# Cognoscan/entropy_coders

Hardware: AMD Instinct MI355X
Metric: FSE encode+decode GiB/s on 1 GiB synthetic bytes; bit-exact round-trip (higher is better)
Workload: dtype u8

## Files before the change

entropy_coders_amd/csrc/fse_decode.hip:

```cpp
#include <type_traits>
#include <utility>

#include "fse_device.hpp"
#include "fse_kernels.h"


namespace fsehip {

__device__ uint32_t g_rank_fb_dec;
hipError_t rank_fallbacks_dec(uint32_t* out, bool reset) {
    hipError_t e = hipMemcpyFromSymbol(out, HIP_SYMBOL(g_rank_fb_dec), 4, 0, hipMemcpyDeviceToHost);
    if (e == hipSuccess && reset) {
        const uint32_t z = 0;
        e = hipMemcpyToSymbol(HIP_SYMBOL(g_rank_fb_dec), &z, 4, 0, hipMemcpyHostToDevice);
    }
    return e;
}

constexpr int STAGE_AUX = 2;

template <int LMAX>
struct Dte {
    static constexpr uint32_t SH = LMAX > 14 ? 17u : 18u;
    __device__ static __forceinline__ uint32_t make(uint32_t nb, uint32_t sym, uint32_t ns) {
        return nb | (sym << 8) | (ns << SH);
    }
    __device__ static __forceinline__ uint32_t ns(uint32_t e) { return e >> SH; }
};
__device__ __forceinline__ uint32_t dte_nb(uint32_t e) { return e & 0xFFu; }
__device__ __forceinline__ uint32_t dte_sym(uint32_t e) { return (e >> 8) & 0xFFu; }

constexpr uint32_t DEC_GROUP = 32;

struct WindowReader {
    const uint32_t* w;
    uint64_t buf;
    int32_t base;
    int32_t pos;
    __device__ __forceinline__ void init(const uint32_t* words, int32_t p) {
        w = words;
        pos = p;
        base = ((p + 31) & ~31) - 64;
        if (base < 0) base = 0;
        buf = (uint64_t)w[base >> 5] | ((uint64_t)w[(base >> 5) + 1] << 32);
    }
    __device__ __forceinline__ uint32_t pop(uint32_t nb) {
        pos -= (int32_t)nb;
        return (uint32_t)(buf >> (uint32_t)(pos - base)) & ((1u << nb) - 1u);
    }
    __device__ __forceinline__ void refill() {
        if (pos - base < 32 && base > 0) {
            base -= 32;
            buf = (buf << 32) | (uint64_t)w[base >> 5];
        }
    }
};

__device__ __forceinline__ bool ckpt_match(uint64_t e, int32_t hdr_bits, uint32_t smask, int32_t pos, uint32_t a0,
                                           uint32_t a1) {
    return (int32_t)(uint32_t)e + hdr_bits == pos && ((((uint32_t)(e >> 32) & smask) << 2) == a0) &&
           ((((uint32_t)(e >> 48) & smask) << 2) == a1);
}

template <int LMAX, class Ent, class Pop>
__device__ __forceinline__ int32_t finish2(uint32_t o, uint32_t n, uint32_t& s0, uint32_t& s1, int32_t& pos,
                                           int32_t hdr_bits, uint8_t* __restrict__ out, Ent ent, Pop pop) {
    for (;;) {
        if (o + 2u == n) {
            out[o++] = (uint8_t)dte_sym(ent(s0));
            out[o++] = (uint8_t)dte_sym(ent(s1));
            break;
        }
        if (o + 1u == n) {
            out[o++] = (uint8_t)dte_sym(ent(s0));
            break;
        }
        const uint32_t e0 = ent(s0);
        uint32_t nb = dte_nb(e0);
        if (pos - (int32_t)nb < hdr_bits) {
            out[o++] = (uint8_t)dte_sym(e0);
            if (o < n) out[o++] = (uint8_t)dte_sym(ent(s1));
            break;
        }
        s0 = Dte<LMAX>::ns(e0) + pop(nb);
        out[o++] = (uint8_t)dte_sym(e0);
        const uint32_t e1 = ent(s1);
        nb = dte_nb(e1);
        if (pos - (int32_t)nb < hdr_bits) {
            out[o++] = (uint8_t)dte_sym(e1);
            if (o < n) out[o++] = (uint8_t)dte_sym(ent(s0));
            break;
        }
        s1 = Dte<LMAX>::ns(e1) + pop(nb);
        out[o++] = (uint8_t)dte_sym(e1);
    }
    return o != n ? FSE_ERR_LENGTH_MISMATCH : pos == hdr_bits ? FSE_OK : FSE_ERR_BAD_SIDECAR;
}

template <int LMAX>
__device__ __forceinline__ int32_t decode_segment(WindowReader& br, uint32_t& s0, uint32_t& s1, uint32_t p0,
                                                  uint32_t p1, bool last, uint32_t n, uint32_t Pm,
                                                  uint8_t* __restrict__ out, const uint32_t* dt, int32_t hdr_bits) {
    uint32_t p = p0;
    for (; p + 8u <= p1; p += 8u) {
        uint32_t w[4];
#pragma unroll
        for (int j = 0; j < 8; ++j) {
            const uint32_t e0 = dt[s0], e1 = dt[s1];
            const uint32_t v0 = br.pop(dte_nb(e0));
            const uint32_t v1 = br.pop(dte_nb(e1));
            s0 = Dte<LMAX>::ns(e0) + v0;
            s1 = Dte<LMAX>::ns(e1) + v1;
            const uint32_t pr = __builtin_amdgcn_perm(e1, e0, 0x0c0c0501u);
            if (j & 1) w[j >> 1] |= pr << 16; else w[j >> 1] = pr;
            br.refill();
        }
        *reinterpret_cast<uint4*>(out + 2u * p) = make_uint4(w[0], w[1], w[2], w[3]);
    }
    for (; p < p1; ++p) {
        const uint32_t e0 = dt[s0], e1 = dt[s1];
        const uint32_t v0 = br.pop(dte_nb(e0));
        const uint32_t v1 = br.pop(dte_nb(e1));
        s0 = Dte<LMAX>::ns(e0) + v0;
        s1 = Dte<LMAX>::ns(e1) + v1;
        out[2u * p] = (uint8_t)dte_sym(e0);
        out[2u * p + 1u] = (uint8_t)dte_sym(e1);
        br.refill();
    }
    if (!last) return FSE_OK;
    return finish2<LMAX>(2u * Pm, n, s0, s1, br.pos, hdr_bits, out, [&](uint32_t s) { return dt[s]; },
                         [&](uint32_t nb) {
                             const uint32_t v = br.pop(nb);
                             br.refill();
                             return v;
                         });
}

template <int LMAX>
__device__ __forceinline__ int32_t decode_segment1(WindowReader& br, uint32_t& s, uint32_t p, uint32_t p1, bool last,
                                                   uint32_t n, uint8_t* __restrict__ out, const uint32_t* dt,
                                                   int32_t hdr_bits) {
    for (; p < p1; ++p) {
        const uint32_t e = dt[s];
        s = Dte<LMAX>::ns(e) + br.pop(dte_nb(e));
        br.refill();
        out[p] = (uint8_t)dte_sym(e);
    }
    if (!last) return FSE_OK;
    out[n - 1u] = (uint8_t)dte_sym(dt[s]);
    return br.pos == hdr_bits ? FSE_OK : FSE_ERR_BAD_SIDECAR;
}

constexpr int32_t PAIR_MAX_BITS = 28;
struct LdsChain {
    int32_t pos, B;
    uint32_t whi, wlo, a0, a1;
    __device__ __forceinline__ void init(const uint32_t* pay, int32_t p, uint32_t s0, uint32_t s1) {
        pos = p;
        a0 = s0 << 2;
        a1 = s1 << 2;
        B = (p - PAIR_MAX_BITS) & ~31;
        wlo = 0;
        whi = *reinterpret_cast<const uint32_t*>(reinterpret_cast<const uint8_t*>(pay) + (B >> 3) + 4);
    }
    __device__ __forceinline__ uint32_t pair(const uint32_t* pay, const uint8_t* dtb) {
        const int32_t lo = (pos - PAIR_MAX_BITS) & ~31;
        const uint32_t w0 = *reinterpret_cast<const uint32_t*>(reinterpret_cast<const uint8_t*>(pay) + (lo >> 3));
        const uint32_t e0 = *reinterpret_cast<const uint32_t*>(dtb + a0);
        const uint32_t e1 = *reinterpret_cast<const uint32_t*>(dtb + a1);
        const uint32_t w1 = lo == B ? whi : wlo;
        pos -= (int32_t)((e0 + e1) & 0xFFu);
        const uint32_t x = (uint32_t)((((uint64_t)w1 << 32) | w0) >> (uint32_t)(pos - lo));
        B = lo;
        whi = w1;
        wlo = w0;
        const uint32_t v1 = __builtin_amdgcn_ubfe(x, 0u, e1);
        const uint32_t v0 = __builtin_amdgcn_ubfe(x, e1, e0);
        a0 = (e0 >> 16) + (v0 << 2);
        a1 = (e1 >> 16) + (v1 << 2);
        return __builtin_amdgcn_perm(e1, e0, 0x0c0c0501u);
    }
    __device__ __forceinline__ uint32_t s0() const { return a0 >> 2; }
    __device__ __forceinline__ uint32_t s1() const { return a1 >> 2; }
    __device__ static __forceinline__ uint32_t entry(const uint8_t* dtb, uint32_t s) {
        return *reinterpret_cast<const uint32_t*>(dtb + 4u * s);
    }
};
template <class Chain, class Tab>
__device__ __forceinline__ uint32_t two_pairs(Chain& c, const uint32_t* pay, const Tab& dtb) {
    const uint32_t lo = c.pair(pay, dtb);
    const uint32_t hi = c.pair(pay, dtb);
    return __builtin_amdgcn_perm(hi, lo, 0x05040100u);
}
__device__ __forceinline__ uint32_t lds_bits32(const uint32_t* pay, int32_t pos) {
    const uint32_t* wp = pay + ((uint32_t)pos >> 5);
    return __builtin_amdgcn_alignbit(wp[1], wp[0], (uint32_t)pos);
}

__device__ __forceinline__ void store_group(uint8_t* __restrict__ dst, const uint32_t* w) {
    uint4* o4 = reinterpret_cast<uint4*>(dst);
#pragma unroll
    for (uint32_t q = 0; q < DEC_GROUP / 8u; ++q) o4[q] = make_uint4(w[4 * q], w[4 * q + 1], w[4 * q + 2], w[4 * q + 3]);
}

__device__ __forceinline__ void rows_transpose(uint32_t* w) {
#pragma unroll
    for (int c = 0; c < 2; ++c)
#pragma unroll
        for (int d = 0; d < 4; ++d) {
            const auto r = __builtin_amdgcn_permlane32_swap(w[4 * c + d], w[4 * (c + 2) + d], false, false);
            w[4 * c + d] = r[0];
            w[4 * (c + 2) + d] = r[1];
        }
#pragma unroll
    for (int c = 0; c < 4; c += 2)
#pragma unroll
        for (int d = 0; d < 4; ++d) {
            const auto r = __builtin_amdgcn_permlane16_swap(w[4 * c + d], w[4 * (c + 1) + d], false, false);
            w[4 * c + d] = r[0];
            w[4 * (c + 1) + d] = r[1];
        }
}

template <class Chain, class Tab>
__device__ __forceinline__ void run_groups_tx(Chain& c, uint32_t my_ng, uint32_t ng_max, const uint32_t* pay,
                                              const Tab& dtb, uint8_t* const* obase, const uint32_t* ong,
                                              uint32_t row) {
    for (uint32_t g = 0; g < ng_max; ++g) {
        uint32_t w[DEC_GROUP / 2u];
        if (g < my_ng) {
#pragma unroll
            for (uint32_t j = 0; j < DEC_GROUP; j += 2u) w[j >> 1] = two_pairs(c, pay, dtb);
        } else {
#pragma unroll
            for (uint32_t j = 0; j < DEC_GROUP / 2u; ++j) w[j] = 0;
        }
        rows_transpose(w);
#pragma unroll
        for (int k = 0; k < 4; ++k)
            if (g < ong[k])
                __builtin_nontemporal_store(u32x4{w[4 * k], w[4 * k + 1], w[4 * k + 2], w[4 * k + 3]},
                                            reinterpret_cast<u32x4*>(obase[k] + g * 2u * DEC_GROUP + 16u * row));
    }
}

template <class Chain, class Tab>
__device__ __forceinline__ void run_chains2(Chain& a, Chain& b, const uint32_t* pay, const Tab& dtb, uint32_t pa,
                                            uint32_t pb, uint32_t ng, uint8_t* __restrict__ out) {
    for (uint32_t g = 0; g < ng; ++g) {
        uint32_t wa[DEC_GROUP / 2u], wb[DEC_GROUP / 2u];
#pragma unroll
        for (uint32_t j = 0; j < DEC_GROUP; j += 2u) {
            const uint32_t la = a.pair(pay, dtb);
            const uint32_t lb = b.pair(pay, dtb);
            const uint32_t ha = a.pair(pay, dtb);
            const uint32_t hb = b.pair(pay, dtb);
            wa[j >> 1] = __builtin_amdgcn_perm(ha, la, 0x05040100u);
            wb[j >> 1] = __builtin_amdgcn_perm(hb, lb, 0x05040100u);
        }
        store_group(out + 2u * (pa + g * DEC_GROUP), wa);
        store_group(out + 2u * (pb + g * DEC_GROUP), wb);
    }
}

template <class Chain, class Tab>
__device__ __forceinline__ int32_t run_chain(Chain& c, const uint32_t* pay, const Tab& dtb, uint32_t p, uint32_t p1,
                                             bool last, uint32_t n, uint32_t Pm, uint8_t* __restrict__ out,
                                             int32_t hdr_bits) {
    for (; p + DEC_GROUP <= p1; p += DEC_GROUP) {
        uint32_t w[DEC_GROUP / 2u];
#pragma unroll
        for (uint32_t j = 0; j < DEC_GROUP; j += 2u) w[j >> 1] = two_pairs(c, pay, dtb);
        store_group(out + 2u * p, w);
    }
    for (; p < p1; ++p) {
        const uint32_t pr = c.pair(pay, dtb);
        out[2u * p] = (uint8_t)pr;
        out[2u * p + 1u] = (uint8_t)(pr >> 8);
    }
    if (!last) return FSE_OK;
    uint32_t s0 = c.s0(), s1 = c.s1();
    return finish2<11>(2u * Pm, n, s0, s1, c.pos, hdr_bits, out, [&](uint32_t s) { return Chain::entry(dtb, s); },
                       [&](uint32_t nb) {
                           c.pos -= (int32_t)nb;
                           return __builtin_amdgcn_ubfe(lds_bits32(pay, c.pos), 0u, nb);
                       });
}

struct LdsChain1 {
    int32_t pos;
    uint32_t Q, whi, wlo, a;
    __device__ __forceinline__ void init(const uint32_t* pay, int32_t p, uint32_t s) {
        pos = p;
        a = s << 2;
        Q = ((uint32_t)p >> 3) & ~3u;
        wlo = 0;
        whi = *reinterpret_cast<const uint32_t*>(reinterpret_cast<const uint8_t*>(pay) + Q);
    }
    __device__ __forceinline__ uint32_t window(const uint32_t* pay) {
        const uint32_t q = ((uint32_t)pos >> 3) & ~3u;
        const uint32_t wq = *reinterpret_cast<const uint32_t*>(reinterpret_cast<const uint8_t*>(pay) + q - 4u);
        const uint32_t hi = q == Q ? whi : wlo;
        Q = q;
        whi = hi;
        wlo = wq;
        return __builtin_amdgcn_alignbit(hi, wq, (uint32_t)pos);
    }
    __device__ __forceinline__ uint32_t step(const uint32_t* pay, const uint8_t* dtb) {
        const uint32_t e = *reinterpret_cast<const uint32_t*>(dtb + a);
        const uint32_t x = window(pay);
        pos -= (int32_t)(e & 0xFFu);
        a = (e >> 16) + (__builtin_amdgcn_ubfe(x, 0u - e, e) << 2);
        return e;
    }
    __device__ __forceinline__ uint32_t pair(const uint32_t* pay, const uint8_t* dtb) {
        const uint32_t e0 = *reinterpret_cast<const uint32_t*>(dtb + a);
        const uint32_t x = window(pay);
        const uint32_t o0 = 0u - e0;
        const uint32_t a1 = (e0 >> 16) + (__builtin_amdgcn_ubfe(x, o0, e0) << 2);
        const uint32_t e1 = *reinterpret_cast<const uint32_t*>(dtb + a1);
        a = (e1 >> 16) + (__builtin_amdgcn_ubfe(x, o0 - e1, e1) << 2);
        pos -= (int32_t)((e0 + e1) & 0xFFu);
        return __builtin_amdgcn_perm(e1, e0, 0x0c0c0501u);
    }
};
struct Chain1x2 {
    LdsChain1 c;
    __device__ __forceinline__ uint32_t pair(const uint32_t* pay, const uint8_t* dtb) { return c.pair(pay, dtb); }
};

__device__ __forceinline__ int32_t run_chain1(LdsChain1& c, const uint32_t* pay, const uint8_t* dtb, uint32_t p,
                                              uint32_t p1, bool last, uint32_t n, uint8_t* __restrict__ out,
                                              int32_t hdr_bits) {
    constexpr uint32_t G = 2u * DEC_GROUP;
    for (; p + G <= p1; p += G) {
        uint32_t w[G / 4u];
#pragma unroll
        for (uint32_t j = 0; j < G; j += 4u) {
            const uint32_t lo = c.pair(pay, dtb), hi = c.pair(pay, dtb);
            w[j >> 2] = __builtin_amdgcn_perm(hi, lo, 0x05040100u);
        }
        uint4* o4 = reinterpret_cast<uint4*>(out + p);
#pragma unroll
        for (uint32_t q = 0; q < G / 16u; ++q) o4[q] = make_uint4(w[4 * q], w[4 * q + 1], w[4 * q + 2], w[4 * q + 3]);
    }
    for (; p < p1; ++p) out[p] = (uint8_t)dte_sym(c.step(pay, dtb));
    if (!last) return FSE_OK;
    out[n - 1u] = (uint8_t)dte_sym(*reinterpret_cast<const uint32_t*>(dtb + c.a));
    return c.pos == hdr_bits ? FSE_OK : FSE_ERR_BAD_SIDECAR;
}

template <uint32_t NT = 256u>
__device__ __forceinline__ uint32_t seg_of(uint32_t tid) {
    return (tid * 33u) & (NT - 1u);
}

template <int LMAX, uint32_t PMAX, uint32_t NW = 4u>
struct PreSmem {
    uint32_t pad[4];
    uint32_t pay[PMAX / 4];
    uint32_t dt[1u << LMAX];
    int err[NW];
};

template <int LMAX, uint32_t PMAX, int NS, uint32_t NT, class Smem>
__device__ __forceinline__ void decode_pre_block(const DecParams& P, Smem& sm, const uint64_t gb) {
    constexpr bool BIG = LMAX > 14;
    constexpr uint32_t NW = NT / 64u;
    const uint32_t tid = threadIdx.x, lane = tid & 63u, wv = tid >> 6;
    if (gb >= P.n_blocks) return;
    const uint8_t* in = P.in + gb * P.slot_bytes;
    const uint32_t clen = P.comp_len[gb];
    const uint64_t ooff = gb * (uint64_t)P.block_size;
    const uint32_t n = (uint32_t)min((uint64_t)P.block_size, P.n_total - ooff);
    uint8_t* out = P.out + ooff;
    const int32_t info = P.dtinfo[gb];
    const bool in_lds = !BIG && clen <= PMAX;
    if (P.pass >= 2 && P.status[gb] != FSE_DEFERRED) return;
    FSE_STAMP(P, 0);
    if (info < 0 || n < (NS == 2 ? 2u : 1u)) {
        if (tid == 0) P.status[gb] = info < 0 ? info : FSE_ERR_LENGTH_MISMATCH;
        return;
    }
    if ((P.pass == 1 || P.pass == 3) && !in_lds) {
        if (tid == 0) P.status[gb] = FSE_DEFERRED;
        return;
    }
    const int32_t hdr_bits = (info & 0xFFFF) * 8;
    const uint32_t L = (uint32_t)info >> 16;
    {
        if (in_lds) {
            const uint32_t nvec = (clen + 15u) >> 4;
            const uint4* src4 = reinterpret_cast<const uint4*>(in);
            uint4* dst4 = reinterpret_cast<uint4*>(sm.pay);
            for (uint32_t i = wv * 64u; i < nvec; i += NT)
                if (i + lane < nvec) __builtin_amdgcn_global_load_lds(src4 + i + lane, dst4 + i, 16, 0, STAGE_AUX);
        }
        {
            const uint32_t dvec = 1u << L >> 2;
            const uint4* t4 = reinterpret_cast<const uint4*>(P.dt + gb * (uint64_t)(1u << LMAX));
            uint4* d4 = reinterpret_cast<uint4*>(sm.dt);
            for (uint32_t i = wv * 64u; i < dvec; i += NT)
                if (i + lane < dvec) __builtin_amdgcn_global_load_lds(t4 + i + lane, d4 + i, 16, 0, STAGE_AUX);
        }
        asm volatile("s_waitcnt vmcnt(0)" ::: "memory");
        __syncthreads();
    }
    FSE_STAMP(P, 3);
    const uint32_t smask = (1u << L) - 1u;
    const uint32_t Pm = NS == 2 ? ((n & 1u) ? (n - 3u) / 2u : n / 2u - 1u) : n - 1u;
    const uint32_t I = P.ckpt_interval;
    const uint32_t nseg = Pm / I + 1u;
    const uint64_t* sc = P.sidecar + gb * P.ckpt_per_block;
    const uint32_t maxbp = clen * 8u - (uint32_t)hdr_bits;
    using Chain = LdsChain;
    const uint8_t* dtb = reinterpret_cast<const uint8_t*>(sm.dt);
    const uint32_t* gw = reinterpret_cast<const uint32_t*>(in);
    int32_t err = FSE_OK;
    uint32_t base0 = 0;
    if (NS == 2 && !BIG && in_lds && NT <= 256u) {
        for (; base0 + NT < nseg; base0 += 2u * NT) {
            const uint32_t sa = base0 + seg_of<NT>(tid), sb = sa + NT;
            bool act[2] = {sa < nseg, sb < nseg};
            const uint32_t sg[2] = {sa, sb};
            Chain c[2];
            uint32_t pp[2], pe[2];
            uint64_t en[2];
            int32_t r[2] = {FSE_OK, FSE_OK};
#pragma unroll
            for (int k = 0; k < 2; ++k) {
                pp[k] = sg[k] * I;
                pe[k] = min(pp[k] + I, Pm);
                en[k] = 0;
                if (!act[k]) continue;
                const uint64_t e = sc[sg[k]];
                en[k] = sg[k] == nseg - 1u ? 0ull : sc[sg[k] + 1u];
                if ((uint32_t)e > maxbp) {
                    r[k] = FSE_ERR_BAD_SIDECAR;
                    act[k] = false;
                    continue;
                }
                c[k].init(sm.pay, hdr_bits + (int32_t)(uint32_t)e, (uint32_t)(e >> 32) & smask,
                          (uint32_t)(e >> 48) & smask);
            }
            const uint32_t ng = (act[0] && act[1]) ? min(pe[0] - pp[0], pe[1] - pp[1]) / DEC_GROUP : 0u;
            run_chains2(c[0], c[1], sm.pay, dtb, pp[0], pp[1], ng, out);
#pragma unroll
            for (int k = 0; k < 2; ++k) {
                if (!act[k]) continue;
                const bool last = sg[k] == nseg - 1u;
                r[k] = run_chain(c[k], sm.pay, dtb, pp[k] + ng * DEC_GROUP, pe[k], last, n, Pm, out, hdr_bits);
                if (r[k] == FSE_OK && !last &&
                    !ckpt_match(en[k], hdr_bits, smask, c[k].pos, c[k].s0() << 2, c[k].s1() << 2))
                    r[k] = FSE_ERR_BAD_SIDECAR;
            }
            if (r[0] != FSE_OK) err = r[0];
            if (r[1] != FSE_OK) err = r[1];
        }
    }
    if (NS == 2 && !BIG && in_lds) {
        for (; base0 < nseg; base0 += NT) {
            const uint32_t seg = base0 + seg_of<NT>(tid);
            bool act = seg < nseg;
            const uint32_t p0 = seg * I, p1 = act ? min(p0 + I, Pm) : p0;
            const bool lastseg = seg == nseg - 1u;
            int32_t r = FSE_OK;
            Chain c;
            uint64_t en = 0;
            if (act) {
                const uint64_t e = sc[seg];
                en = lastseg ? 0ull : sc[seg + 1u];
                if ((uint32_t)e > maxbp) {
                    r = FSE_ERR_BAD_SIDECAR;
                    act = false;
                } else {
                    c.init(sm.pay, hdr_bits + (int32_t)(uint32_t)e, (uint32_t)(e >> 32) & smask,
                           (uint32_t)(e >> 48) & smask);
                }
            }
            const uint32_t my_ng = act ? (p1 - p0) / DEC_GROUP : 0u;
            const uint32_t ng_max = wave_max(my_ng);
            if (ng_max) {
                uint8_t* obase[4];
                uint32_t ong[4];
#pragma unroll
                for (uint32_t k = 0; k < 4; ++k) {
                    const uint32_t os = base0 + seg_of<NT>((tid & ~63u) + 16u * k + (tid & 15u));
                    const uint32_t oq = os * I;
                    ong[k] = os < nseg ? (min(oq + I, Pm) - oq) / DEC_GROUP : 0u;
                    obase[k] = out + 2u * oq;
                }
                run_groups_tx(c, my_ng, ng_max, sm.pay, dtb, obase, ong, (tid >> 4) & 3u);
            }
            if (act) {
                r = run_chain(c, sm.pay, dtb, p0 + my_ng * DEC_GROUP, p1, lastseg, n, Pm, out, hdr_bits);
                if (r == FSE_OK && !lastseg && !ckpt_match(en, hdr_bits, smask, c.pos, c.s0() << 2, c.s1() << 2))
                    r = FSE_ERR_BAD_SIDECAR;
            }
            if (r != FSE_OK) err = r;
        }
    }
    if (NS == 1 && !BIG && in_lds) {
        constexpr uint32_t G1 = 2u * DEC_GROUP;
        for (; base0 < nseg; base0 += NT) {
            const uint32_t seg = base0 + seg_of<NT>(tid);
            bool act = seg < nseg;
            const uint32_t p0 = seg * I, p1 = act ? min(p0 + I, Pm) : p0;
            const bool lastseg = seg == nseg - 1u;
            int32_t r = FSE_OK;
            Chain1x2 c;
            uint64_t en = 0;
            if (act) {
                const uint64_t e = sc[seg];
                en = lastseg ? 0ull : sc[seg + 1u];
                if ((uint32_t)e > maxbp) {
                    r = FSE_ERR_BAD_SIDECAR;
                    act = false;
                } else {
                    c.c.init(sm.pay, hdr_bits + (int32_t)(uint32_t)e, (uint32_t)(e >> 32) & smask);
                }
            }
            const uint32_t my_ng = act ? (p1 - p0) / G1 : 0u;
            const uint32_t ng_max = wave_max(my_ng);
            if (ng_max) {
                uint8_t* obase[4];
                uint32_t ong[4];
#pragma unroll
                for (uint32_t k = 0; k < 4; ++k) {
                    const uint32_t os = base0 + seg_of<NT>((tid & ~63u) + 16u * k + (tid & 15u));
                    const uint32_t oq = os * I;
                    ong[k] = os < nseg ? (min(oq + I, Pm) - oq) / G1 : 0u;
                    obase[k] = out + oq;
                }
                run_groups_tx(c, my_ng, ng_max, sm.pay, dtb, obase, ong, (tid >> 4) & 3u);
            }
            if (act) {
                r = run_chain1(c.c, sm.pay, dtb, p0 + my_ng * G1, p1, lastseg, n, out, hdr_bits);
                if (r == FSE_OK && !lastseg && !ckpt_match(en, hdr_bits, smask, c.c.pos, c.c.a, 0u))
                    r = FSE_ERR_BAD_SIDECAR;
            }
            if (r != FSE_OK) err = r;
        }
    }
    for (uint32_t base = base0; base < nseg; base += NT) {
        const uint32_t seg = base + (NS == 2 ? seg_of<NT>(tid) : tid);
        if (seg >= nseg) continue;
        const uint64_t e = sc[seg];
        const uint32_t p0 = seg * I, p1 = min(p0 + I, Pm);
        const uint32_t bp = (uint32_t)e;
        uint32_t s0 = (uint32_t)(e >> 32) & smask, s1 = NS == 2 ? (uint32_t)(e >> 48) & smask : 0u;
        const bool lastseg = seg == nseg - 1u;
        const uint64_t en = lastseg ? 0ull : sc[seg + 1u];
        int32_t r;
        if (bp > maxbp) {
            r = FSE_ERR_BAD_SIDECAR;
        } else if (NS == 1) {
            if (!BIG && in_lds) {
                LdsChain1 c;
                c.init(sm.pay, hdr_bits + (int32_t)bp, s0);
                r = run_chain1(c, sm.pay, dtb, p0, p1, lastseg, n, out, hdr_bits);
                if (r == FSE_OK && !lastseg && !ckpt_match(en, hdr_bits, smask, c.pos, c.a, 0u)) r = FSE_ERR_BAD_SIDECAR;
            } else {
                WindowReader br;
                br.init(gw, hdr_bits + (int32_t)bp);
                r = decode_segment1<LMAX>(br, s0, p0, p1, lastseg, n, out, sm.dt, hdr_bits);
                if (r == FSE_OK && !lastseg && !ckpt_match(en, hdr_bits, smask, br.pos, s0 << 2, 0u))
                    r = FSE_ERR_BAD_SIDECAR;
            }
        } else if (!BIG && in_lds) {
            Chain c;
            c.init(sm.pay, hdr_bits + (int32_t)bp, s0, s1);
            r = run_chain(c, sm.pay, dtb, p0, p1, lastseg, n, Pm, out, hdr_bits);
            if (r == FSE_OK && !lastseg && !ckpt_match(en, hdr_bits, smask, c.pos, c.a0, c.a1)) r = FSE_ERR_BAD_SIDECAR;
        } else {
            WindowReader br;
            br.init(gw, hdr_bits + (int32_t)bp);
            r = decode_segment<LMAX>(br, s0, s1, p0, p1, lastseg, n, Pm, out, sm.dt, hdr_bits);
            if (r == FSE_OK && !lastseg && !ckpt_match(en, hdr_bits, smask, br.pos, s0 << 2, s1 << 2))
                r = FSE_ERR_BAD_SIDECAR;
        }
        if (r != FSE_OK) err = r;
    }
    err = -(int32_t)wave_max((uint32_t)(-err));
    if (lane == 0) sm.err[wv] = err;
    __syncthreads();
    FSE_STAMP(P, 4);
    if (tid == 0) {
        int32_t e2 = FSE_OK;
        for (uint32_t w = 0; w < NW; ++w)
            if (sm.err[w] != FSE_OK) e2 = sm.err[w];
        P.status[gb] = e2;
        if (P.out_len) P.out_len[gb] = e2 ? 0u : n;
    }
}

template <int LMAX, uint32_t PMAX, int NS, int PASS, uint32_t NT = 256u>
__global__ __launch_bounds__(NT) void decode_pre_kernel(DecParams P) {
    constexpr bool BIG = LMAX > 14;
    constexpr uint32_t NW = NT / 64u;
    __shared__ PreSmem<LMAX, BIG ? 16u : PMAX, NW> sm;
    if constexpr (PASS <= 1) {
        decode_pre_block<LMAX, PMAX, NS, NT>(P, sm, blockIdx.x);
    } else {
        __shared__ uint64_t dmask[NW];
        const uint32_t tid = threadIdx.x, lane = tid & 63u, wv = tid >> 6;
        const uint64_t G = gridDim.x;
        for (uint64_t r0 = blockIdx.x; r0 < P.n_blocks; r0 += G * NT) {
            const uint64_t gb = r0 + G * tid;
            const bool d = gb < P.n_blocks && P.status[gb] == FSE_DEFERRED;
            const uint64_t m = __ballot(d);
            if (lane == 0) dmask[wv] = m;
            __syncthreads();
            for (uint32_t w = 0; w < NW; ++w) {
                for (uint64_t mw = dmask[w]; mw; mw &= mw - 1u)
                    decode_pre_block<LMAX, PMAX, NS, NT>(P, sm, r0 + G * (64u * w + (uint32_t)__builtin_ctzll(mw)));
            }
            __syncthreads();
        }
    }
}

constexpr uint32_t HP_BLOCKS = 16;
template <int LMAX>
__global__ __launch_bounds__(64) void hdr_parse_kernel(DtParams P) {
    static_assert(LMAX <= 12, "headers of L <= 12 fit the 512 staged bytes");
    constexpr uint32_t NB = HP_BLOCKS;
    __shared__ uint32_t rows[NB][128];
    __shared__ uint32_t nrm[NB][128];
    const uint32_t lane = threadIdx.x;
    const uint64_t gb0 = (uint64_t)blockIdx.x * NB;
    const uint64_t gl = gb0 + lane;
    const bool mine = lane < NB && gl < P.n_blocks;
    const uint32_t clen_l = mine ? P.comp_len[gl] : 0u;
    const uint32_t nw_l = (uint32_t)min((uint64_t)min(clen_l, HDR_MAX) + 3u, P.slot_bytes) >> 2;
    for (uint32_t i = lane; i < NB * 128u; i += 64u) (&nrm[0][0])[i] = 0u;
    uint32_t a[NB], b[NB];
#pragma unroll
    for (uint32_t j = 0; j < NB; ++j) {
        const uint32_t nw = (uint32_t)__builtin_amdgcn_readlane((int)nw_l, (int)j);
        const uint32_t* w = reinterpret_cast<const uint32_t*>(P.in + (gb0 + j) * P.slot_bytes);
        a[j] = lane < nw ? w[lane] : 0u;
        b[j] = lane + 64u < nw ? w[lane + 64u] : 0u;
    }
#pragma unroll
    for (uint32_t j = 0; j < NB; ++j) {
        rows[j][(lane + j) & 127u] = a[j];
        rows[j][(lane + 64u + j) & 127u] = b[j];
    }
    __syncthreads();
    if (mine) {
        uint32_t L = 0, tl = 0;
        typedef __attribute__((address_space(3))) int16_t lds_i16;
        const int hl = header_read_row((const lds_u32*)&rows[lane][0], lane, nw_l, clen_l, (uint32_t)LMAX,
                                       (lds_i16*)&nrm[lane][0], &L, &tl);
        P.hdr_meta[gl] = make_int2(hl, (int)(L | (tl << 8)));
    }
    __syncthreads();
#pragma unroll
    for (uint32_t j = 0; j < NB; ++j) {
        const uint64_t g = gb0 + j;
        if (g >= P.n_blocks) break;
        P.hdr_norm[g * 128u + lane] = nrm[j][(lane + j) & 127u];
        P.hdr_norm[g * 128u + 64u + lane] = nrm[j][(lane + 64u + j) & 127u];
    }
}

template <int LMAX>
__global__ __launch_bounds__(64) void dtable_blocks_kernel(DtParams P) {
    constexpr uint32_t SIZE = 1u << LMAX;
    __shared__ int32_t norm[256];
    __shared__ __attribute__((aligned(16))) uint8_t sym_at[SIZE];
    constexpr uint32_t RKN = LMAX <= 12 ? SIZE : SIZE / 2u + 768u;
    __shared__ __attribute__((aligned(16))) uint16_t rk[RKN];
    static_assert(SIZE + 256 * 4 + 256 * 2 <= RKN * 2, "rank table must cover occ, cnt and cumul");
    uint8_t* occ = reinterpret_cast<uint8_t*>(rk);
    uint32_t* cnt = reinterpret_cast<uint32_t*>(reinterpret_cast<uint8_t*>(rk) + SIZE);
    uint16_t* cumul = reinterpret_cast<uint16_t*>(reinterpret_cast<uint8_t*>(rk) + SIZE + 1024);
    const uint32_t lane = lane_id();
    const uint64_t gb = blockIdx.x;
    if (gb >= P.n_blocks) return;
    FSE_STAMP(P, 0);
    const uint8_t* in = P.in + gb * P.slot_bytes;
    const uint32_t clen = P.comp_len[gb];
    const uint32_t last = (clen && clen <= P.slot_bytes) ? in[clen - 1u] : 0u;
    uint32_t L = 0, tl = 0;
    int hl;
    if (LMAX <= 12 && P.hdr_meta) {
        const int2 m = P.hdr_meta[gb];
        const uint32_t q0 = P.hdr_norm[gb * 128u + lane], q1 = P.hdr_norm[gb * 128u + 64u + lane];
        norm[2u * lane] = (int32_t)(int16_t)(q0 & 0xFFFFu);
        norm[2u * lane + 1u] = (int32_t)(int16_t)(q0 >> 16);
        norm[128u + 2u * lane] = (int32_t)(int16_t)(q1 & 0xFFFFu);
        norm[128u + 2u * lane + 1u] = (int32_t)(int16_t)(q1 >> 16);
        hl = m.x;
        L = (uint32_t)m.y & 0xFFu;
        tl = (uint32_t)m.y >> 8;
        wave_sync();
        FSE_STAMP(P, 1);
        FSE_STAMP(P, 2);
    } else {
        const uint32_t* w = reinterpret_cast<const uint32_t*>(in);
        uint32_t r0, r1;
        if (P.slot_bytes >= HDR_MAX) {
            r0 = w[lane];
            r1 = w[lane + 64u];
        }
        const uint32_t nw = (uint32_t)min((uint64_t)min(clen, HDR_MAX) + 3u, P.slot_bytes) >> 2;
        if (P.slot_bytes < HDR_MAX) {
            r0 = lane < nw ? w[lane] : 0u;
            r1 = lane + 64u < nw ? w[lane + 64u] : 0u;
        }
        r0 = lane < nw ? r0 : 0u;
        r1 = lane + 64u < nw ? r1 : 0u;
        for (uint32_t s = lane; s < 256u; s += WAVE) norm[s] = 0;
        wave_sync();
        FSE_STAMP(P, 1);
        hl = header_read_wave(r0, r1, clen, (uint32_t)LMAX, norm, &L, &tl);
        FSE_STAMP(P, 2);
    }
    int rc = hl < 0 ? hl : FSE_OK;
    if (rc == FSE_OK && ((uint32_t)hl >= clen || last == 0)) rc = FSE_ERR_NO_MARKER;
    if (rc == FSE_OK && clen > (1u << 28)) rc = FSE_ERR_UNSUPPORTED;
    wave_sync();
    if (rc == FSE_OK) {
        const uint32_t size = 1u << L;
        uint32_t* dt = P.dt + gb * (uint64_t)SIZE;
        auto visit = [&](uint32_t i, uint32_t s, uint32_t nx) {
            const uint32_t nb = L - ilog2u(nx);
            dt[i] = Dte<LMAX>::make(nb, s, (nx << nb) - size);
        };
        auto first_x = [&](uint32_t s) {
            const int32_t v = norm[s];
            return v < 0 ? 1u : (uint32_t)v;
        };
        const RankAtomic ra{P.peer_ranks == 0u, occ, nullptr, 0u, &g_rank_fb_dec, P.rank_inject};
        if (LMAX <= 12)
            rc = wave_build_spread<SIZE / 64u, true>(norm, L, tl, sym_at, occ, cumul, cnt, visit, first_x, ra, rk,
                                                     nullptr, &P);
        else rc = wave_build_spread<64, true>(norm, L, tl, sym_at, occ, cumul, cnt, visit, first_x, ra);
    }
    FSE_STAMP(P, 8);
    if (lane == 0) P.dtinfo[gb] = rc == FSE_OK ? (int32_t)((uint32_t)hl | (L << 16)) : rc;
}


template <int LMAX>
__global__ __launch_bounds__(64) void decode1_serial_kernel(DecParams P) {
    const uint64_t gb = blockIdx.x;
    if (gb >= P.n_blocks) return;
    const int32_t info = P.dtinfo[gb];
    uint32_t nbor = 0;
    if (info >= 0) {
        const uint32_t* t = P.dt + gb * (uint64_t)(1u << LMAX);
        for (uint32_t i = threadIdx.x; i < (1u << ((uint32_t)info >> 16)); i += 64u) nbor |= t[i] & 0xFFu;
    }
    const bool single = __ballot(nbor != 0u) == 0ull;
    if (threadIdx.x != 0) return;
    if (info < 0) {
        P.status[gb] = info;
        if (P.out_len) P.out_len[gb] = 0;
        return;
    }
    const uint8_t* in = P.in + gb * P.slot_bytes;
    const uint32_t clen = P.comp_len[gb];
    const int32_t hdr_bits = (info & 0xFFFF) * 8;
    const uint32_t L = (uint32_t)info >> 16;
    const uint32_t* dt = P.dt + gb * (uint64_t)(1u << LMAX);
    uint8_t* out = P.out + gb * (uint64_t)P.block_size;
    const bool known = P.n_total != 0;
    const uint32_t n = known ? (uint32_t)min((uint64_t)P.block_size, P.n_total - gb * (uint64_t)P.block_size) : 0u;
    const uint32_t cap = known ? n : P.out_cap;
    int32_t err = FSE_OK;
    uint32_t o = 0;
    const int32_t top = (int32_t)(clen - 1u) * 8 + (int32_t)ilog2u(in[clen - 1]);
    WindowReader br;
    br.init(reinterpret_cast<const uint32_t*>(in), top);
    if (br.pos - (int32_t)L < hdr_bits) {
        err = FSE_ERR_TOO_SHORT;
    } else {
        uint32_t s = br.pop(L);
        br.refill();
        for (;;) {
            if (known && single && o + 1u >= n) break;
            const uint32_t e = dt[s];
            const uint32_t nb = dte_nb(e);
            if (br.pos - (int32_t)nb < hdr_bits) break;
            if (o >= cap) {
                err = single ? FSE_ERR_SINGLE_SYMBOL : FSE_ERR_DST_TOO_SMALL;
                break;
            }
            s = Dte<LMAX>::ns(e) + br.pop(nb);
            br.refill();
            out[o++] = (uint8_t)dte_sym(e);
        }
        if (err == FSE_OK) {
            if (o >= cap) err = FSE_ERR_DST_TOO_SMALL;
            else out[o++] = (uint8_t)dte_sym(dt[s]);
        }
        if (known && (err == FSE_ERR_DST_TOO_SMALL || (err == FSE_OK && o != n))) err = FSE_ERR_LENGTH_MISMATCH;
    }
    P.status[gb] = err;
    if (P.out_len) P.out_len[gb] = err ? 0u : o;
}

struct ChunkReader {
    const uint4* w4;
    uint64_t buf;
    int32_t base, pos;
    uint4 cl, ch, nl, nh;
    int32_t c;
    __device__ __forceinline__ void init(const uint8_t* in, int32_t p) {
        w4 = reinterpret_cast<const uint4*>(in);
        const uint32_t* w = reinterpret_cast<const uint32_t*>(in);
        pos = p;
        base = max(((p + 31) & ~31) - 64, 0);
        buf = (uint64_t)w[base >> 5] | ((uint64_t)w[(base >> 5) + 1] << 32);
        c = ((base >> 5) - 1) >> 3;
        cl = w4[2 * max(c, 0)];
        ch = w4[2 * max(c, 0) + 1];
        nl = w4[2 * max(c - 1, 0)];
        nh = w4[2 * max(c - 1, 0) + 1];
    }
    __device__ __forceinline__ uint32_t pop(uint32_t nb) {
        pos -= (int32_t)nb;
        return (uint32_t)(buf >> (uint32_t)(pos - base)) & ((1u << nb) - 1u);
    }
    __device__ __forceinline__ void refill() {
        if (pos - base < 32 && base > 0) {
            base -= 32;
            const int32_t wi = base >> 5;
            if ((wi >> 3) != c) {
                cl = nl;
                ch = nh;
                c -= 1;
                nl = w4[2 * max(c - 1, 0)];
                nh = w4[2 * max(c - 1, 0) + 1];
            }
            const uint32_t j = (uint32_t)wi & 7u;
            const uint4 q = j < 4u ? cl : ch;
            const uint32_t k = j & 3u;
            const uint32_t v = k == 0 ? q.x : k == 1 ? q.y : k == 2 ? q.z : q.w;
            buf = (buf << 32) | v;
        }
    }
};

template <int LMAX>
__global__ __launch_bounds__(64) void serial2_decode_kernel(DecParams P) {
    __shared__ uint32_t tab[1u << LMAX];
    const uint64_t gb = blockIdx.x;
    if (gb >= P.n_blocks) return;
    const int32_t info = P.dtinfo[gb];
    const uint32_t lane = threadIdx.x;
    uint32_t nbor = 0;
    if (info >= 0) {
        const uint32_t nv = (1u << ((uint32_t)info >> 16)) >> 2;
        const uint4* t4 = reinterpret_cast<const uint4*>(P.dt + gb * (uint64_t)(1u << LMAX));
        uint4* d4 = reinterpret_cast<uint4*>(tab);
        for (uint32_t i = lane; i < nv; i += 64u) {
            const uint4 q = t4[i];
            d4[i] = q;
            nbor |= (q.x | q.y | q.z | q.w) & 0xFFu;
        }
    }
    const bool single = __ballot(nbor != 0u) == 0ull;
    __syncthreads();
    if (lane != 0) return;
    const uint8_t* in = P.in + gb * P.slot_bytes;
    const uint32_t clen = P.comp_len[gb];
    const bool known = P.n_total != 0;
    const uint64_t ooff = gb * (uint64_t)P.block_size;
    const uint32_t n = known ? (uint32_t)min((uint64_t)P.block_size, P.n_total - ooff) : 0u;
    const uint32_t lim = known ? n : P.out_cap;
    uint8_t* out = P.out + ooff;
    int32_t err = info < 0 ? info : FSE_OK;
    if (err == FSE_OK && known && n < 2) err = FSE_ERR_LENGTH_MISMATCH;
    if (err == FSE_OK && !known && single) err = FSE_ERR_SINGLE_SYMBOL;
    const int32_t hdr_bits = (info & 0xFFFF) * 8;
    const uint32_t L = (uint32_t)info >> 16;
    uint32_t o = 0;
    if (err == FSE_OK) {
        const int32_t top = (int32_t)(clen - 1u) * 8 + (int32_t)ilog2u(in[clen - 1]);
        if (top - 2 * (int32_t)L < hdr_bits) err = FSE_ERR_TOO_SHORT;
    }
    if (err == FSE_OK) {
        ChunkReader br;
        br.init(in, (int32_t)(clen - 1u) * 8 + (int32_t)ilog2u(in[clen - 1]));
        uint32_t s0 = br.pop(L);
        br.refill();
        uint32_t s1 = br.pop(L);
        br.refill();
        const uint32_t I = P.ckpt_interval;
        uint64_t* rec = (P.sidecar_out && I) ? P.sidecar_out + gb * P.ckpt_per_block : nullptr;
        const uint32_t ckmask = I ? I - 1u : 0u;
        uint32_t pidx = 0;
        auto record = [&]() {
            if (rec && (pidx & ckmask) == 0u && pidx / I < P.ckpt_per_block)
                rec[pidx / I] = (uint64_t)(uint32_t)(br.pos - hdr_bits) | ((uint64_t)s0 << 32) | ((uint64_t)s1 << 48);
        };
        while (o + 18u < lim && br.pos - hdr_bits >= 16 * (int32_t)L) {
// ... 932 lines not shown
```

Before: 514.3.

## Fold segment tails into transposed group loop and set waves-per-EU from LDS

Each segment's partial final group is now decoded inside the wave-cooperative transposed group loop, with byte-granular partial stores. This replaces the separate scalar per-segment tail pass, which was divergent. The decode kernel also gets an amdgpu_waves_per_eu attribute computed from the LDS footprint, so the register budget matches the occupancy that LDS allows. The cost is a ballot-guarded slow path with per-byte stores whenever any lane in the wave has a tail, and possible register pressure changes.

Measured after the change: 520.3 (median of 6 runs). 1.2% higher.

```diff
diff --git a/entropy_coders_amd/csrc/fse_decode.hip b/entropy_coders_amd/csrc/fse_decode.hip
--- a/entropy_coders_amd/csrc/fse_decode.hip
+++ b/entropy_coders_amd/csrc/fse_decode.hip
@@ -153,6 +153,7 @@
 
 constexpr int32_t PAIR_MAX_BITS = 28;
 struct LdsChain {
+    static constexpr bool SINGLE_STEP = false;
     int32_t pos, B;
     uint32_t whi, wlo, a0, a1;
     __device__ __forceinline__ void init(const uint32_t* pay, int32_t p, uint32_t s0, uint32_t s1) {
@@ -222,13 +223,58 @@
         }
 }
 
+__device__ __forceinline__ void store_chunk(uint8_t* __restrict__ dst, const uint32_t* t, uint32_t nb) {
+    if (nb >= 16u) {
+        __builtin_nontemporal_store(u32x4{t[0], t[1], t[2], t[3]}, reinterpret_cast<u32x4*>(dst));
+        return;
+    }
+#pragma unroll
+    for (uint32_t i = 0; i < 4u; ++i) {
+        if (nb >= 4u * i + 4u) {
+            *reinterpret_cast<uint32_t*>(dst + 4u * i) = t[i];
+        } else if (nb > 4u * i) {
+            dst[4u * i] = (uint8_t)t[i];
+            if (nb > 4u * i + 1u) dst[4u * i + 1u] = (uint8_t)(t[i] >> 8);
+            if (nb > 4u * i + 2u) dst[4u * i + 2u] = (uint8_t)(t[i] >> 16);
+        }
+    }
+}
+
 template <class Chain, class Tab>
-__device__ __forceinline__ void run_groups_tx(Chain& c, uint32_t my_ng, uint32_t ng_max, const uint32_t* pay,
-                                              const Tab& dtb, uint8_t* const* obase, const uint32_t* ong,
-                                              uint32_t row) {
+__device__ __forceinline__ void run_groups_tx(Chain& c, uint32_t my_ng, uint32_t tail, uint32_t ng_max,
+                                              const uint32_t* pay, const Tab& dtb, uint8_t* __restrict__ out,
+                                              const uint32_t* obase, const uint32_t* ong, uint32_t row,
+                                              uint32_t own_off) {
     for (uint32_t g = 0; g < ng_max; ++g) {
         uint32_t w[DEC_GROUP / 2u];
-        if (g < my_ng) {
+        const bool part = g == my_ng && tail != 0u;
+        if (__ballot(part) != 0ull) {
+            const uint32_t nb = g < my_ng ? 2u * DEC_GROUP : part ? tail : 0u;
+#pragma unroll
+            for (uint32_t j = 0; j < DEC_GROUP / 2u; ++j) w[j] = 0;
+#pragma unroll 1
+            for (uint32_t q = 0; q < 4u; ++q) {
+                const uint32_t lim = nb > 16u * q ? nb - 16u * q : 0u;
+                const uint32_t cnt = lim >> 1;
+                uint32_t t[4];
+#pragma unroll
+                for (uint32_t j = 0; j < 8u; j += 2u) {
+                    uint32_t x = 0;
+                    if (j < cnt) x = c.pair(pay, dtb);
+                    if (j + 1u < cnt) x = __builtin_amdgcn_perm(c.pair(pay, dtb), x, 0x05040100u);
+                    if constexpr (Chain::SINGLE_STEP) {
+                        if ((lim & 1u) && j == cnt) x = c.step_sym(pay, dtb);
+                        if ((lim & 1u) && j + 1u == cnt) x |= c.step_sym(pay, dtb) << 16;
+                    }
+                    t[j >> 1] = x;
+                }
+                if (part && lim) store_chunk(out + (own_off + g * 2u * DEC_GROUP + 16u * q), t, lim);
+#pragma unroll
+                for (uint32_t i = 0; i < DEC_GROUP / 2u - 4u; ++i) w[i] = w[i + 4u];
+#pragma unroll
+                for (uint32_t i = 0; i < 4u; ++i) w[DEC_GROUP / 2u - 4u + i] = t[i];
+            }
+        } else if (g < my_ng) {
 #pragma unroll
             for (uint32_t j = 0; j < DEC_GROUP; j += 2u) w[j >> 1] = two_pairs(c, pay, dtb);
         } else {
@@ -239,8 +285,9 @@
 #pragma unroll
         for (int k = 0; k < 4; ++k)
             if (g < ong[k])
-                __builtin_nontemporal_store(u32x4{w[4 * k], w[4 * k + 1], w[4 * k + 2], w[4 * k + 3]},
-                                            reinterpret_cast<u32x4*>(obase[k] + g * 2u * DEC_GROUP + 16u * row));
+                __builtin_nontemporal_store(
+                    u32x4{w[4 * k], w[4 * k + 1], w[4 * k + 2], w[4 * k + 3]},
+                    reinterpret_cast<u32x4*>(out + (obase[k] + g * 2u * DEC_GROUP + 16u * row)));
     }
 }
 
@@ -325,8 +372,12 @@
     }
 };
 struct Chain1x2 {
+    static constexpr bool SINGLE_STEP = true;
     LdsChain1 c;
     __device__ __forceinline__ uint32_t pair(const uint32_t* pay, const uint8_t* dtb) { return c.pair(pay, dtb); }
+    __device__ __forceinline__ uint32_t step_sym(const uint32_t* pay, const uint8_t* dtb) {
+        return dte_sym(c.step(pay, dtb));
+    }
 };
 
 __device__ __forceinline__ int32_t run_chain1(LdsChain1& c, const uint32_t* pay, const uint8_t* dtb, uint32_t p,
@@ -479,21 +530,22 @@
                 }
             }
             const uint32_t my_ng = act ? (p1 - p0) / DEC_GROUP : 0u;
-            const uint32_t ng_max = wave_max(my_ng);
+            const uint32_t tail = act ? 2u * ((p1 - p0) % DEC_GROUP) : 0u;
+            const uint32_t ng_max = wave_max(my_ng + (tail ? 1u : 0u));
             if (ng_max) {
-                uint8_t* obase[4];
+                uint32_t obase[4];
                 uint32_t ong[4];
 #pragma unroll
                 for (uint32_t k = 0; k < 4; ++k) {
                     const uint32_t os = base0 + seg_of<NT>((tid & ~63u) + 16u * k + (tid & 15u));
                     const uint32_t oq = os * I;
                     ong[k] = os < nseg ? (min(oq + I, Pm) - oq) / DEC_GROUP : 0u;
-                    obase[k] = out + 2u * oq;
+                    obase[k] = 2u * oq;
                 }
-                run_groups_tx(c, my_ng, ng_max, sm.pay, dtb, obase, ong, (tid >> 4) & 3u);
+                run_groups_tx(c, my_ng, tail, ng_max, sm.pay, dtb, out, obase, ong, (tid >> 4) & 3u, 2u * p0);
             }
             if (act) {
-                r = run_chain(c, sm.pay, dtb, p0 + my_ng * DEC_GROUP, p1, lastseg, n, Pm, out, hdr_bits);
+                r = run_chain(c, sm.pay, dtb, p1, p1, lastseg, n, Pm, out, hdr_bits);
                 if (r == FSE_OK && !lastseg && !ckpt_match(en, hdr_bits, smask, c.pos, c.s0() << 2, c.s1() << 2))
                     r = FSE_ERR_BAD_SIDECAR;
             }
@@ -521,21 +573,22 @@
                 }
             }
             const uint32_t my_ng = act ? (p1 - p0) / G1 : 0u;
-            const uint32_t ng_max = wave_max(my_ng);
+            const uint32_t tail = act ? (p1 - p0) % G1 : 0u;
+            const uint32_t ng_max = wave_max(my_ng + (tail ? 1u : 0u));
             if (ng_max) {
-                uint8_t* obase[4];
+                uint32_t obase[4];
                 uint32_t ong[4];
 #pragma unroll
                 for (uint32_t k = 0; k < 4; ++k) {
                     const uint32_t os = base0 + seg_of<NT>((tid & ~63u) + 16u * k + (tid & 15u));
                     const uint32_t oq = os * I;
                     ong[k] = os < nseg ? (min(oq + I, Pm) - oq) / G1 : 0u;
-                    obase[k] = out + oq;
+                    obase[k] = oq;
                 }
-                run_groups_tx(c, my_ng, ng_max, sm.pay, dtb, obase, ong, (tid >> 4) & 3u);
+                run_groups_tx(c, my_ng, tail, ng_max, sm.pay, dtb, out, obase, ong, (tid >> 4) & 3u, p0);
             }
             if (act) {
-                r = run_chain1(c.c, sm.pay, dtb, p0 + my_ng * G1, p1, lastseg, n, out, hdr_bits);
+                r = run_chain1(c.c, sm.pay, dtb, p1, p1, lastseg, n, out, hdr_bits);
                 if (r == FSE_OK && !lastseg && !ckpt_match(en, hdr_bits, smask, c.c.pos, c.c.a, 0u))
                     r = FSE_ERR_BAD_SIDECAR;
             }
@@ -594,8 +647,16 @@
     }
 }
 
+template <class Smem>
+constexpr uint32_t lds_waves_per_simd(uint32_t nw) {
+    const uint32_t w = (160u << 10) / (uint32_t)sizeof(Smem) * nw / 4u;
+    return w < 1u ? 1u : w > 8u ? 8u : w;
+}
+
 template <int LMAX, uint32_t PMAX, int NS, int PASS, uint32_t NT = 256u>
-__global__ __launch_bounds__(NT) void decode_pre_kernel(DecParams P) {
+__global__ __launch_bounds__(NT) __attribute__((amdgpu_waves_per_eu(
+    lds_waves_per_simd<PreSmem<LMAX, (LMAX > 14) ? 16u : PMAX, NT / 64u>>(NT / 64u)))) void
+decode_pre_kernel(DecParams P) {
     constexpr bool BIG = LMAX > 14;
     constexpr uint32_t NW = NT / 64u;
     __shared__ PreSmem<LMAX, BIG ? 16u : PMAX, NW> sm;
```
